# EavianWoo/SinGS

Hardware: AMD Instinct MI355X
Metric: rendered views/sec fwd+bwd, 200k Gaussians @1080p (higher is better)
Workload: dtype f32; 1 GPU; S(200000,1920,1080,deg=3,seed=3): 200000 Gaussians, 1920x1080, SH deg 3, fwd+bwd, R=780064 (tile,Gaussian) pairs, every view of a step within 0.1 % of that (cameras a few cm apart), frame-parallel dp1; gaussians=200000, width=1920, height=1080, sh_degree=3, num_rendered=780064, tile_list_max=135, frames_per_launch=8, streams=2, regularisers=False, forward_only=False, hip_graph=False, reduction=fold of 2 gradient row(s) for 16 views + collective in 1 chunk(s), gradient_rows=2, parallelism=dp1

## Files before the change

include/sings_hip.h:

```cpp
#ifndef SINGS_HIP_H
#define SINGS_HIP_H

#include <stddef.h>
#include <stdint.h>

#ifdef __cplusplus
extern "C" {
#endif

#define SG_TILE 16
#define SG_GRAD_REC_FLOATS 9

typedef struct SgRasterSettings {
    int32_t image_height;
    int32_t image_width;
    float tanfovx;
    float tanfovy;
    float scale_modifier;
    int32_t sh_degree;
    int32_t sh_coeffs;
    int32_t prefiltered;
    int32_t debug;
    int32_t flags;
    const float *bg;
// ... 347 lines not shown
int sg_init_attributes(int V, int F, int E, float init_scale_multiplier, float thickness_factor, const float *verts,
                       const int32_t *faces, const int32_t *edges, void *ws, int32_t *first, int32_t *second, float *scales,
                       float *scales_aux, float *normals, float *rotmat, int32_t *info, void *stream);
size_t sg_attr_mse_ws_bytes(void);
int sg_attr_mse(int N, const float *const *outputs, const float *const *targets, float *const *grads, void *ws, float *terms,
                void *stream);
int sg_plateau_step(int n_groups, int begin, int patience, const double *settings, const float *loss, double *state, float *hyper,
                    const float *terms, int n_copy, double *log, int log_rows, void *stream);

#define SG_NUM_KERNELS 8
enum SgKernelId {
    SG_K_PREPROCESS_FWD = 0, SG_K_PHOTO_LOSS = 1, SG_K_TILE_SCAN = 2, SG_K_TILE_SCATTER = 3,
    SG_K_TILE_SORT = 4, SG_K_RENDER_FWD = 5, SG_K_RENDER_BWD = 6, SG_K_PREPROCESS_BWD = 7
};
int sg_profile_enable(int on);
int sg_copy_probe(void *dst, const void *src, size_t bytes, int non_temporal, void *stream);
int sg_profile_collect(double *total_ms, int64_t *launches, int n);
const char *sg_kernel_name(int id);

#ifdef __cplusplus
}
#endif
#endif
```

sings_amd/_lib.py:

```python
import ctypes as C
import os

_HERE = os.path.dirname(os.path.abspath(__file__))
LIB_PATH = os.environ.get("SINGS_HIP_LIB") or os.path.join(_HERE, "libsings_hip.so")
_lib = None


class SgRasterSettings(C.Structure):
    _fields_ = [
        ("image_height", C.c_int32), ("image_width", C.c_int32),
        ("tanfovx", C.c_float), ("tanfovy", C.c_float), ("scale_modifier", C.c_float),
        ("sh_degree", C.c_int32), ("sh_coeffs", C.c_int32),
        ("prefiltered", C.c_int32), ("debug", C.c_int32), ("flags", C.c_int32),
        ("bg", C.c_void_p), ("viewmatrix", C.c_void_p), ("projmatrix", C.c_void_p), ("campos", C.c_void_p),
        ("count_signal", C.c_void_p), ("count_signal_host", C.c_void_p),
    ]


class SgLayout(C.Structure):
    _fields_ = [(n, C.c_size_t) for n in (
        "geom_recA", "geom_recB", "geom_recC", "geom_depth", "geom_flags", "geom_slot", "geom_bytes",
        "bin_header", "bin_tile_count", "bin_ranges", "bin_cursor", "bin_pair_keys", "bin_point_list",
        "bin_point_keys", "bin_pair_gid", "bin_pair_tile", "bin_pair_local", "bin_sort_items", "bin_rank_items", "bin_items", "bin_ck_start", "bin_plan", "bin_pair_mask", "bin_item_w", "bin_item_perm", "bin_rec_valid", "bin_tile_keys", "bin_bytes", "img_final_T", "img_n_contrib", "img_ckpt", "img_bytes", "bwd_bytes")]

# ... 115 lines not shown
    "sg_mesh_edges_build": "i: i2 p5",
    "sg_mesh_edges_emit": "i: i3 p7",
    "sg_mesh_subdivide": "i: i3 p6",
    "sg_mesh_midpoints": "i: i3 p4",
    "sg_mesh_midpoints_i32": "i: i3 p4",
    "sg_mesh_collapse_max_edges": "i:",
    "sg_mesh_collapse_ws_bytes": "z: i2",
    "sg_mesh_collapse_build": "i: i3 p3 d p3",
    "sg_mesh_collapse_emit": "i: i4 p6",
    "sg_init_ws_bytes": "z: i",
    "sg_init_attributes": "i: i3 f2 p12",
    "sg_attr_mse_ws_bytes": "z:",
    "sg_attr_mse": "i: i V3 p3",
    "sg_plateau_step": "i: i3 d p4 i p i p",
    "sg_profile_enable": "i: i",
    "sg_copy_probe": "i: p2 z i p",
    "sg_profile_collect": "i: d n i",
    "sg_kernel_name": "s: i",
}
_P = C.POINTER
_CTYPE = {"i": C.c_int, "z": C.c_size_t, "f": C.c_float, "s": C.c_char_p,
          "p": C.c_void_p,
          "S": _P(SgRasterSettings), "F": _P(SgFrameBatch), "K": _P(SgSkinInputs), "L": _P(SgLayout), "T": _P(SgTriplane),
          "D": _P(SgLinearSide),
          "n": _P(C.c_int64), "Z": _P(C.c_size_t), "d": _P(C.c_double),
          "V": _P(C.c_void_p),
          "G": _P(C.c_void_p * 3 * 4)}
EXPORTS = tuple(_PROTOTYPES)
LPIPS_NUM_OFFSETS = 46
LPIPS_WS_NUM_PIECES = 28
# ... 64 lines not shown
```

sings_amd/csrc/sg_api.hip:

```cpp
#include "sg_common.h"

#include <chrono>
#include <stdarg.h>
#include <stdio.h>
#include <stdlib.h>
#include <thread>
#include <string.h>
#include <utility>
#include <vector>

static thread_local char g_err[512] = "";

static int sg_fail(const char *what, hipError_t e)
{
    snprintf(g_err, sizeof g_err, "%s: %s", what, e == hipSuccess ? "invalid argument" : hipGetErrorString(e));
    return 1;
}

static int sg_failf(const char *fmt, ...)
{
    char msg[256];
    va_list ap;
    va_start(ap, fmt);
    vsnprintf(msg, sizeof msg, fmt, ap);
// ... 1153 lines not shown
    if (!g_prof_on) return;
    hipEvent_t e;
    (void)hipEventCreate(&e);
    (void)hipEventRecord(e, st);
    g_prof_open[id] = e;
}
void sg_prof_end(int id, hipStream_t st)
{
    if (!g_prof_on) return;
    hipEvent_t e;
    (void)hipEventCreate(&e);
    (void)hipEventRecord(e, st);
    g_prof_ev[id].push_back(std::make_pair(g_prof_open[id], e));
}
extern "C" int sg_profile_enable(int on) { g_prof_on = on != 0; return 0; }
extern "C" int sg_profile_collect(double *total_ms, int64_t *launches, int n)
{
    if (!total_ms || !launches || n < SG_NUM_KERNELS) return sg_fail("sg_profile_collect", hipSuccess);
    hipError_t e = hipDeviceSynchronize();
    if (e != hipSuccess) return sg_fail("sg_profile_collect", e);
    for (int k = 0; k < SG_NUM_KERNELS; k++) {
        for (auto &p : g_prof_ev[k]) {
            float ms = 0;
            (void)hipEventElapsedTime(&ms, p.first, p.second);
            total_ms[k] += ms; launches[k] += 1;
            (void)hipEventDestroy(p.first); (void)hipEventDestroy(p.second);
        }
        g_prof_ev[k].clear();
    }
    return 0;
// ... 9 lines not shown
```

sings_amd/csrc/sg_common.h:

```cpp
#pragma once
#include <hip/hip_runtime.h>
#include <stdint.h>
#include <stddef.h>

#include "../../include/sings_hip.h"

#define SG_WAVE 64
int sg_set_error(const char *what, hipError_t e = hipSuccess);
#ifdef SG_EXP
#error "SG_EXP experiment variants were removed from the product sources"
#endif
#define SG_MAX_TILES (1u << 20)
#define SG_SEG 256
__host__ __device__ inline uint32_t sg_nseg(uint32_t n) { return n > SG_SEG && n <= SG_SEG * 4095u ? (n + SG_SEG - 1) / SG_SEG : 0u; }
__host__ __device__ inline uint32_t sg_items_cap(size_t T, size_t cap) { size_t v = T + cap / SG_SEG + 2; return v > 0xffffffffull ? 0xffffffffu : (uint32_t)v; }
__host__ __device__ inline uint32_t sg_group_slots(uint32_t n) { return n > 1024u ? 6u * ((n + 1023u) / 1024u) + 2u : 0u; }
__host__ __device__ inline uint32_t sg_sort_items_cap(size_t T, size_t cap) { size_t v = (T < cap / 1024 ? T : cap / 1024) + 2; return v > 0xffffffffull ? 0xffffffffu : (uint32_t)v; }
__host__ __device__ inline uint32_t sg_rank_items_cap(size_t cap) { size_t v = cap / 73 + 16; return v > 0xffffffffull ? 0xffffffffu : (uint32_t)v; }
__host__ __device__ inline uint32_t sg_ckpt_cap(size_t cap) { size_t v = 2 * (cap / SG_SEG) + 2; return v > 0xffffffffull ? 0xffffffffu : (uint32_t)v; }
__host__ __device__ inline uint32_t sg_ctr_blocks_x(uint32_t gx) { return (gx + 3u) >> 2; }
__host__ __device__ inline size_t sg_ctr_count(uint32_t gx, uint32_t gy) { return (size_t)sg_ctr_blocks_x(gx) * ((gy + 3u) >> 2) * 16u; }
__host__ __device__ inline uint32_t sg_ctr_index(uint32_t tx, uint32_t ty, uint32_t gx)
{
    return ((ty >> 2) * sg_ctr_blocks_x(gx) + (tx >> 2)) * 16u + ((ty & 3u) << 2) + (tx & 3u);
// ... 184 lines not shown
struct SgCam {
    int W, H, gx, gy, flags;
    float tanfovx, tanfovy, fx, fy, mod;
    int D, M;
    const float *view, *proj, *campos, *bg;
    unsigned long long *count_signal;
};
__host__ __device__ __forceinline__ SgCam sg_frame(SgCam c, int frame, int cam_stride)
{
    const size_t f = (size_t)frame * (size_t)cam_stride;
    c.view += 16 * f; c.proj += 16 * f; c.campos += 3 * f;
    if (c.count_signal) c.count_signal += frame;
    return c;
}

void sg_launch_preprocess_fwd(const SgCam &c, const SgBatch &bt, int P, const float *means3D, const float *shs,
                              const float *colors_precomp, const float *opacities, const float *scales,
                              const float *rotations, const float *cov3D_precomp, SgGeom g, SgBin b,
                              size_t cap, int32_t *radii, hipStream_t st);
void sg_launch_binning(const SgCam &c, const SgBatch &bt, int P, const int32_t *radii, SgGeom g, SgBin b, size_t cap,
                       int write_keys, hipStream_t st);
static inline uint32_t sg_cap32(size_t cap) { return cap > 0xffffffffull ? 0xffffffffu : (uint32_t)cap; }
void sg_launch_render_fwd(const SgCam &c, const SgBatch &bt, SgGeom g, SgBin b, size_t cap, SgImg im, float *out_color,
                          int write_keys, hipStream_t st, const SgAuxFwd *ax = nullptr);
void sg_launch_render_bwd(const SgCam &c, const SgBatch &bt, SgGeom g, SgBin b, size_t cap, SgImg im,
                          const float *dL_dpix, SgRec grec, hipStream_t st, const SgAuxBwd *ax = nullptr);
void sg_launch_record_sums(const SgBatch &bt, int P, const int32_t *radii, SgGeom g, SgRec grec, size_t cap, const uint32_t *header,
                           const uint8_t *rec_valid, float4 *a9out, hipStream_t st, const float *dz = nullptr, size_t dz_stride = 0);
static inline size_t sg_a9_bytes(int P, int K) { return K > 1 ? sg_align((size_t)K * (size_t)P * 48 + 256) : 0; }
void sg_launch_preprocess_bwd(const SgCam &c, const SgBatch &bt, int P, const float *means3D, const float *shs,
// ... 77 lines not shown
```

sings_amd/csrc/sg_render.hip:

```cpp
#include "sg_sort.h"

#define SG_FB 256
#define SG_BB 64
#define SG_UNSET 0xffffffffu

__device__ __forceinline__ float sg_exp(float x) { return __builtin_amdgcn_exp2f(x * 1.44269504088896340736f); }
#define SG_KA (-0.5f * 1.44269504088896340736f)
#define SG_KB (-1.44269504088896340736f)
__device__ __forceinline__ float sg_power2(float Ap, float Bp, float Cp, float dx, float dy)
{
    return fmaf(Cp * dy, dy, fmaf(Ap, dx, Bp * dy) * dx);
}

#define SG_XCD_RUN 16
__device__ __forceinline__ int sg_tile_of_block(int block)
{
    const int xcd = block & 7, slot = block >> 3;
    const int within = (slot + 7 * (slot >> 5)) & (SG_XCD_RUN - 1);
    return ((slot / SG_XCD_RUN) * 8 + xcd) * SG_XCD_RUN + within;
}

__device__ __forceinline__ float sg_min_q_rect(float A, float B, float C, float mx, float my, float x0, float x1,
                                               float y0, float y1)
{
    if (mx >= x0 && mx <= x1 && my >= y0 && my <= y1) return 0.0f;
    const float rA = __builtin_amdgcn_rcpf(A), rC = __builtin_amdgcn_rcpf(C);
    float best = 3.0e38f;
// ... 296 lines not shown

static inline int sg_render_blocks(int T) { return ((T + 8 * SG_XCD_RUN - 1) / (8 * SG_XCD_RUN)) * (8 * SG_XCD_RUN); }

void sg_launch_render_fwd(const SgCam &c, const SgBatch &bt, SgGeom g, SgBin b, size_t cap, SgImg im, float *out_color,
                          int write_keys, hipStream_t st, const SgAuxFwd *ax)
{
    static_assert(SG_FB == SG_SEG, "forward batches are the checkpoint granularity");
    const int T = c.gx * c.gy;
    const int grid = sg_render_blocks(T);
    const int grid4 = sg_render_blocks((T + 3) / 4);
    const unsigned K = (unsigned)bt.K;
    const bool few = sg_lds_hist(c.gx, c.gy);
    uint64_t *pk = write_keys ? b.point_keys : (uint64_t *)nullptr;
    const uint32_t key_pitch = sg_key_pitch(c.gx, c.gy, c.flags);
    const bool direct = key_pitch != 0u;
#define SG_RF_ARGS(NB) c.W, c.H, c.gx, T, NB, b.ranges, direct ? b.tile_keys : b.pair_keys, b.point_list, pk, g.recA, g.recB, g.recC, c.bg, out_color,     \
                       im.final_T, im.n_contrib, b.ck_start, im.ckpt, sg_ckpt_cap(cap), b.header, b.pair_mask, b.tile_count,       \
                       (const uint4 *)b.sort_items, sg_mask_plane(cap), b.plan, b.item_w, sg_items_cap((size_t)T, cap), key_pitch
    sg_prof_begin(SG_K_RENDER_FWD, st);
    if (ax && (K > 1 || (few && (c.flags & SG_FLAG_THROUGHPUT)))) {
        if (few) hipLaunchKernelGGL(sg_render_fwd_frames_aux_kernel<true>, dim3(grid, K), dim3(256), 0, st, bt, SG_RF_ARGS(grid), *ax);
        else hipLaunchKernelGGL(sg_render_fwd_frames_aux_kernel<false>, dim3(grid4, K), dim3(256), 0, st, bt, SG_RF_ARGS(grid4), *ax);
    } else if (ax) {
        if (few) {
            const int extra = sg_split_long(c.gx, c.gy, c.flags) ? 3 * (int)sg_sort_items_cap(T, cap) : 0;
            hipLaunchKernelGGL(sg_render_fwd_deep_aux_kernel, dim3(extra + grid), dim3(256), 0, st, SG_RF_ARGS(extra), *ax);
        } else
            hipLaunchKernelGGL(sg_render_fwd_aux_kernel, dim3(grid), dim3(256), 0, st, SG_RF_ARGS(grid), *ax);
    } else if (K > 1 || (few && (c.flags & SG_FLAG_THROUGHPUT))) {
        if (few) hipLaunchKernelGGL(sg_render_fwd_frames_kernel<true>, dim3(grid, K), dim3(256), 0, st, bt, SG_RF_ARGS(grid));
        else hipLaunchKernelGGL(sg_render_fwd_frames_kernel<false>, dim3(grid4, K), dim3(256), 0, st, bt, SG_RF_ARGS(grid4));
    } else if (few) {
        const int extra = sg_split_long(c.gx, c.gy, c.flags) ? 3 * (int)sg_sort_items_cap(T, cap) : 0;
        hipLaunchKernelGGL(sg_render_fwd_deep_kernel, dim3(extra + grid), dim3(256), 0, st, SG_RF_ARGS(extra));
    } else
        hipLaunchKernelGGL(sg_render_fwd_kernel, dim3(grid), dim3(256), 0, st, SG_RF_ARGS(grid));
    sg_prof_end(SG_K_RENDER_FWD, st);
#undef SG_RF_ARGS
}

#define SG_DPP(v, ctrl) __builtin_bit_cast(float, __builtin_amdgcn_update_dpp(0, __builtin_bit_cast(int, v), ctrl, 0xF, 0xF, false))

__device__ __forceinline__ float sg_reduce9(float v[9], int lane, float *v8tot)
{
    float a0 = v[0], a1 = v[1], a2 = v[2], a3 = v[3], a4 = v[4], a5 = v[5], a6 = v[6], a7 = v[7];
    asm volatile("s_nop 1\n\tv_permlane32_swap_b32 %0, %1\n\tv_permlane32_swap_b32 %2, %3\n\t"
// ... 20 lines not shown
}
__device__ __forceinline__ float sg_reduce_to63(float x)
{
    x += SG_DPP(x, 0xB1); x += SG_DPP(x, 0x4E); x += SG_DPP(x, 0x141); x += SG_DPP(x, 0x140);
    asm volatile("s_nop 1\n\tv_add_f32_dpp %0, %0, %0 row_bcast:15 row_mask:0xa\n\ts_nop 1\n\t"
                 "v_add_f32_dpp %0, %0, %0 row_bcast:31 row_mask:0xc" : "+v"(x));
    return x;
}
__device__ __forceinline__ int sg_red_idx(int lane)
{
    const int row = lane >> 4, half = (lane >> 3) & 1;
    const int base = row == 0 ? 0 : (row == 1 ? 2 : (row == 2 ? 1 : 3));
    return base + 4 * half;
}

#define SG_BWD_EVAL(KPOS, SKIP)                                                                                       \
                                     \
    const float dx = ga.x - pxf, dy = ga.y - pyf;                                                                     \
    const float power = sg_power2(ga.z, ga.w, gb.x, dx, dy);            \
    const float G = __builtin_amdgcn_exp2f(power);                                                                    \
    const float alpha = fminf(0.99f, gb.y * G);                                                                       \
    const bool valid = ((KPOS) < ncq_b) & !(power > 0.0f) & !(alpha < 1.0f / 255.0f);                                 \
    if (__ballot(valid) == 0ull) SKIP;                   \
    const float ae = valid ? alpha : 0.0f;                                                                            \
    const float rinv = __builtin_amdgcn_rcpf(1.0f - ae);                                     \
    Tr = Tr * rinv;                                                                     \
    const float dchan = ae * Tr;                                                                                      \
                         \
    const float e = (AUX ? fmaf(gz, dD, fmaf(gc, d2, fmaf(gb.w, d1, gb.z * d0))) : fmaf(gc, d2, fmaf(gb.w, d1, gb.z * d0))) - Sd; \
    Sd = fmaf(ae, e, Sd);                                                                                             \
    const float dLa = fmaf(-tb, rinv, e * Tr);                        \
    const float w = valid ? G * dLa : 0.0f;                          \
         \
          \
    do { } while (0)
#define SG_BWD_PARTIALS(V)                                                                                            \
    const float wx = w * dx, wy = w * dy;                                                                             \
// ... 104 lines not shown
#include "sg_render_bwd.inc"
#undef SG_BWD_AUX
#define SG_BWD_AUX 1
#include "sg_render_bwd.inc"
#undef SG_BWD_AUX

void sg_launch_render_bwd(const SgCam &c, const SgBatch &bt, SgGeom g, SgBin b, size_t cap, SgImg im,
                          const float *dL_dpix, SgRec grec, hipStream_t st, const SgAuxBwd *ax)
{
    static_assert(SG_SEG % SG_BB == 0, "segments are whole backward batches");
    const int T = c.gx * c.gy;
    const int grid = sg_render_blocks((int)sg_items_cap((size_t)T, cap));
    const int grid4 = sg_render_blocks((int)((sg_items_cap((size_t)T, cap) + 3u) / 4u));
    const unsigned K = (unsigned)bt.K;
    uint32_t cap32 = cap > 0xffffffffull ? 0xffffffffu : (uint32_t)cap;
    sg_prof_begin(SG_K_RENDER_BWD, st);
    if (sg_lds_hist(c.gx, c.gy)) {
        hipLaunchKernelGGL(sg_order_items_kernel, dim3(1, K), dim3(256), 0, st, bt, b.header, b.item_w, b.item_perm);
        if (ax)
        hipLaunchKernelGGL(sg_render_bwd_sparse_aux_kernel, dim3(grid, K), dim3(256), 0, st, bt, c.W, c.H, c.gx, T, grid, b.ranges,
                           b.point_list, g.recA, g.recB, g.recC, c.bg, im.final_T, im.n_contrib, dL_dpix,
                           grec.a, grec.b, cap32, b.header, b.items, b.ck_start, im.ckpt, sg_ckpt_cap(cap), b.pair_mask, sg_mask_plane(cap),
                           sg_split_long(c.gx, c.gy, c.flags) ? 1 : 0, b.item_perm, b.rec_valid, *ax);
        else
        hipLaunchKernelGGL(sg_render_bwd_sparse_kernel, dim3(grid, K), dim3(256), 0, st, bt, c.W, c.H, c.gx, T, grid, b.ranges,
                           b.point_list, g.recA, g.recB, g.recC, c.bg, im.final_T, im.n_contrib, dL_dpix,
                           grec.a, grec.b, cap32, b.header, b.items, b.ck_start, im.ckpt, sg_ckpt_cap(cap), b.pair_mask, sg_mask_plane(cap),
                           sg_split_long(c.gx, c.gy, c.flags) ? 1 : 0, b.item_perm, b.rec_valid);
    } else if (ax)
    hipLaunchKernelGGL(sg_render_bwd_aux_kernel, dim3(grid4, K), dim3(256), 0, st, bt, c.W, c.H, c.gx, T, grid4, b.ranges,
                       b.point_list, g.recA, g.recB, g.recC, c.bg, im.final_T, im.n_contrib, dL_dpix,
                       grec.a, grec.b, cap32, b.header, b.items, b.ck_start, im.ckpt, sg_ckpt_cap(cap), b.pair_mask, sg_mask_plane(cap),
                       sg_split_long(c.gx, c.gy, c.flags) ? 1 : 0, *ax);
    else
    hipLaunchKernelGGL(sg_render_bwd_kernel, dim3(grid4, K), dim3(256), 0, st, bt, c.W, c.H, c.gx, T, grid4, b.ranges,
                       b.point_list, g.recA, g.recB, g.recC, c.bg, im.final_T, im.n_contrib, dL_dpix,
                       grec.a, grec.b, cap32, b.header, b.items, b.ck_start, im.ckpt, sg_ckpt_cap(cap), b.pair_mask, sg_mask_plane(cap),
                       sg_split_long(c.gx, c.gy, c.flags) ? 1 : 0);
    sg_prof_end(SG_K_RENDER_BWD, st);
}
```

sings_amd/csrc/sg_render_bwd.inc:

```

#define SG_BWD_FIRST(A0, A1, A2, A3, A4, A5, A6, A7, A8, Wv, DX, DY, DC, C0, C1, C2)                                   \
    "v_mul_f32 " A0 ", " Wv ", " DX "\n\tv_mul_f32 " A1 ", " Wv ", " DY "\n\t"                                          \
    "v_mul_f32 " A2 ", " A0 ", " DX "\n\tv_mul_f32 " A3 ", " A0 ", " DY "\n\tv_mul_f32 " A4 ", " A1 ", " DY "\n\t"       \
    "v_mov_b32 " A5 ", " Wv "\n\t"                                                                                    \
    "v_mul_f32 " A6 ", " DC ", " C0 "\n\tv_mul_f32 " A7 ", " DC ", " C1 "\n\tv_mul_f32 " A8 ", " DC ", " C2 "\n\t"
#define SG_BWD_LATER(A0, A1, A2, A3, A4, A5, A6, A7, A8, T0, T1, Wv, DX, DY, DC, C0, C1, C2)                           \
    "v_mul_f32 " T0 ", " Wv ", " DX "\n\tv_mul_f32 " T1 ", " Wv ", " DY "\n\t"                                          \
    "v_add_f32 " A0 ", " A0 ", " T0 "\n\tv_add_f32 " A1 ", " A1 ", " T1 "\n\t"                                          \
    "v_fmac_f32 " A2 ", " T0 ", " DX "\n\tv_fmac_f32 " A3 ", " T0 ", " DY "\n\tv_fmac_f32 " A4 ", " T1 ", " DY "\n\t"    \
    "v_add_f32 " A5 ", " A5 ", " Wv "\n\t"                                                                            \
    "v_fmac_f32 " A6 ", " DC ", " C0 "\n\tv_fmac_f32 " A7 ", " DC ", " C1 "\n\tv_fmac_f32 " A8 ", " DC ", " C2 "\n\t"
#define SG_BWD_ACC9 "+v"(acc[0]), "+v"(acc[1]), "+v"(acc[2]), "+v"(acc[3]), "+v"(acc[4]), "+v"(acc[5]), "+v"(acc[6]), "+v"(acc[7]), "+v"(acc[8])
#define SG_BWD_ASSIGN()                                                                                               \
    do {                                                                                                              \
        if (AUX)                                                                                                      \
            asm volatile(SG_BWD_FIRST("%0", "%1", "%2", "%3", "%4", "%5", "%6", "%7", "%8", "%10", "%11", "%12", "%13", "%14", "%15", "%16") \
                         "v_mul_f32 %9, %13, %17"                                                                     \
                         : SG_BWD_ACC9, "+v"(acc[9]) : "v"(w), "v"(dx), "v"(dy), "v"(dchan), "v"(d0), "v"(d1), "v"(d2), "v"(dD)); \
        else                                                                                                          \
            asm volatile(SG_BWD_FIRST("%0", "%1", "%2", "%3", "%4", "%5", "%6", "%7", "%8", "%9", "%10", "%11", "%12", "%13", "%14", "%15") \
                         : SG_BWD_ACC9 : "v"(w), "v"(dx), "v"(dy), "v"(dchan), "v"(d0), "v"(d1), "v"(d2));             \
    } while (0)
#define SG_BWD_ASSIGN_OR_ADD()                                                                                        \
    do {                                                                                                              \
// ... 3 lines not shown
                         SG_BWD_LATER("%0", "%1", "%2", "%3", "%4", "%5", "%6", "%7", "%8", "%10", "%11", "%12", "%13", "%14", "%15", "%16", "%17", "%18") \
                         "v_fmac_f32 %9, %15, %19\n\ts_branch 2f\n1:\n\t"                                            \
                         SG_BWD_FIRST("%0", "%1", "%2", "%3", "%4", "%5", "%6", "%7", "%8", "%12", "%13", "%14", "%15", "%16", "%17", "%18") \
                         "v_mul_f32 %9, %15, %19\n2:"                                                                  \
                         : SG_BWD_ACC9, "+v"(acc[9]), "=&v"(t0), "=&v"(t1)                                             \
                         : "v"(w), "v"(dx), "v"(dy), "v"(dchan), "v"(d0), "v"(d1), "v"(d2), "v"(dD), "s"(some) : "scc"); \
        else                                                                                                          \
            asm volatile("s_cmp_lg_u32 %18, 0\n\ts_cbranch_scc0 1f\n\t"                                              \
                         SG_BWD_LATER("%0", "%1", "%2", "%3", "%4", "%5", "%6", "%7", "%8", "%9", "%10", "%11", "%12", "%13", "%14", "%15", "%16", "%17") \
                         "s_branch 2f\n1:\n\t"                                                                        \
                         SG_BWD_FIRST("%0", "%1", "%2", "%3", "%4", "%5", "%6", "%7", "%8", "%11", "%12", "%13", "%14", "%15", "%16", "%17") \
                         "\n2:"                                                                                       \
                         : SG_BWD_ACC9, "=&v"(t0), "=&v"(t1)                                                          \
                         : "v"(w), "v"(dx), "v"(dy), "v"(dchan), "v"(d0), "v"(d1), "v"(d2), "s"(some) : "scc");        \
    } while (0)
#define SG_BWD_QUAD(Q)                                                                                                \
    do {                                                                                                              \
        const float pxf = ((Q) & 1) ? pxf0 + 8.0f : pxf0, pyf = ((Q) >> 1) ? pyf0 + 8.0f : pyf0;                      \
        const float d0 = d04[Q], d1 = d14[Q], d2 = d24[Q], dD = dD4[Q], tb = tb4[Q];                                  \
        const uint32_t ncq_b = ncq4[Q];                                                                               \
        float &Tr = Tr4[Q], &Sd = Sd4[Q];                                                                             \
        SG_BWD_EVAL((uint32_t)pos, break);                            \
        if ((Q) == 0) SG_BWD_ASSIGN(); else SG_BWD_ASSIGN_OR_ADD();                                                   \
        some = 1u;                                                                                                    \
    } while (0)
__global__ void __launch_bounds__(256) __attribute__((amdgpu_waves_per_eu(SG_BWD_TW_WAVES, SG_BWD_TW_WAVES)))
#if SG_BWD_AUX
sg_render_bwd_aux_kernel(SG_BWD_PARAMS, SgAuxBwd ax)
#else
sg_render_bwd_kernel(SG_BWD_PARAMS)
#endif
{
    constexpr bool AUX = SG_BWD_AUX;
#if !SG_BWD_AUX
    const SgAuxBwd ax = { };
#endif
    __shared__ float4 sR[4][SG_BB][4];
    __shared__ float sG[4][SG_BB][9 + AUX];
    SG_STAMP_SCOPE
    SG_BWD_FRAME_OFFSETS;
#if SG_BWD_AUX
    SG_BWD_AUX_FRAME_OFFSETS;
#endif
    (void)T; (void)nblocks;
    const int nitems = header[1] ? 0 : (int)header[5];
    const int tid = threadIdx.x, lane = tid & 63;
    const int wave = __builtin_amdgcn_readfirstlane(tid >> 6);
    const int it = 4 * sg_tile_of_block(blockIdx.x) + wave;
    if (it >= nitems) return;
    const uint32_t item = items[it];
    const int tile = (int)(item & 0xfffffu), seg = (int)(item >> 20);
    const int tx = tile % gx, ty = tile / gx;
    const int X0 = tx * 16, Y0 = ty * 16;
    const uint2 range = ranges[tile];
    const int n = (int)(range.y - range.x);
    const uint32_t cks = ck_start[tile];
    const int lo = seg * SG_SEG;
    const int hi = cks != 0xffffffffu && lo + SG_SEG < n ? lo + SG_SEG : n;
    if (lo >= n) return;
// ... 25 lines not shown
            }
        }
        Tr4[q] = Tr; Sd4[q] = Sd; d04[q] = d0; d14[q] = d1; d24[q] = d2; dD4[q] = dD; ncq4[q] = ncq;
        uint32_t m = ncq;
#pragma unroll
        for (int o = 32; o > 0; o >>= 1) { uint32_t u = __shfl_xor(m, o, 64); m = u > m ? u : m; }
        maxq4[q] = (int)__builtin_amdgcn_readfirstlane(m);
    }
    const int max_contrib = max(max(maxq4[0], maxq4[1]), max(maxq4[2], maxq4[3]));
    const float ddelx_dx = 0.5f * (float)W, ddely_dy = 0.5f * (float)H;
    const int cslot = lane == 63 ? 8 : sg_red_idx(lane);
    float acc[10] = { };
    for (int base = lo + (hi - 1 - lo) / SG_BB * SG_BB; base >= lo; base -= SG_BB) {
        const int cnt = hi - base < SG_BB ? hi - base : SG_BB;
        uint32_t mk = 0u;
        if (lane < cnt) {
            const int e = base + lane;
            const uint32_t gid = point_list[range.x + e];
            if (e < max_contrib) {
                mk = pair_mask[range.x + e];
                if (split_long && n > SG_WSORT_MAX)
                    mk = (mk & 1u) | (pair_mask[(size_t)mask_plane + range.x + e] & 2u) | (pair_mask[2 * (size_t)mask_plane + range.x + e] & 4u) |
                         (pair_mask[3 * (size_t)mask_plane + range.x + e] & 8u);
                mk &= 15u;
            }
            const float4 c4 = recC[SG_REC_STRIDE * (size_t)gid];
            if (mk) {
                const float4 a = recA[SG_REC_STRIDE * (size_t)gid], b = recB[SG_REC_STRIDE * (size_t)gid];
                sR[wave][lane][0] = make_float4(a.x, a.y, SG_KA * a.z, SG_KB * a.w);
                sR[wave][lane][1] = make_float4(SG_KA * b.x, b.y, b.z, b.w);
                sR[wave][lane][2] = make_float4(c4.x, AUX ? ax.depth[gid] : 0.0f, __uint_as_float(mk), 0.0f);
                sR[wave][lane][3] = make_float4(a.z, a.w, b.x, 0.0f);
            }
            const uint32_t goff = __float_as_uint(c4.y), mn = __float_as_uint(c4.z), wh = __float_as_uint(c4.w);
            const int x0 = mn & 0xffff, y0 = mn >> 16, rw = wh & 0xffff;
            sR[wave][lane][3].w = __uint_as_float(goff + (uint32_t)((ty - y0) * rw + (tx - x0)));
        }
        unsigned long long todo = __ballot(mk != 0u);
        unsigned long long filed = 0ull;
        __builtin_amdgcn_s_waitcnt(0xC07F);
        __builtin_amdgcn_wave_barrier();
        while (todo) {
            const int k = 63 - __builtin_clzll(todo);
            todo &= ~(1ull << k);
            const int pos = base + k;
            const float4 ga = sR[wave][k][0], gb = sR[wave][k][1], gm = sR[wave][k][2];
            const float gc = gm.x, gz = gm.y;
            uint32_t mke = __builtin_amdgcn_readfirstlane(__float_as_uint(gm.z));
            if (pos >= maxq4[0]) mke &= ~1u;
            if (pos >= maxq4[1]) mke &= ~2u;
            if (pos >= maxq4[2]) mke &= ~4u;
            if (pos >= maxq4[3]) mke &= ~8u;
            uint32_t some = 0u;
            if (mke & 1u) SG_BWD_QUAD(0);
            if (mke & 2u) SG_BWD_QUAD(1);
            if (mke & 4u) SG_BWD_QUAD(2);
            if (mke & 8u) SG_BWD_QUAD(3);
            __builtin_amdgcn_wave_barrier();
            if (some) {
                SG_BWD_FILE(acc, acc[9], k);
                filed |= 1ull << k;
            }
        }
        __builtin_amdgcn_s_waitcnt(0xC07F);
        __builtin_amdgcn_wave_barrier();
        const float4 cn = sR[wave][lane][3];
        const uint32_t rslot = lane < cnt ? __float_as_uint(cn.w) : 0xffffffffu;
        if (rslot < cap) {
            float4 r0 = make_float4(0.0f, 0.0f, 0.0f, 0.0f), r1 = r0;
            float r2 = 0.0f, r3 = 0.0f;
            if ((filed >> lane) & 1ull) {
                float s[9 + AUX];
#pragma unroll
                for (int q = 0; q < 9 + AUX; q++) s[q] = sG[wave][lane][q];
                const float no = -sR[wave][lane][1].y, nh = 0.5f * no;
                const float m0 = fmaf(cn.x, s[0], cn.y * s[1]), m1 = fmaf(cn.y, s[0], cn.z * s[1]);
                r0 = make_float4(no * ddelx_dx * m0, no * ddely_dy * m1, nh * s[2], nh * s[3]);
                r1 = make_float4(nh * s[4], s[5], s[6], s[7]);
                r2 = s[8];
                if (AUX) r3 = s[9];
            }
            grec_a[2 * (size_t)rslot] = r0;
            grec_a[2 * (size_t)rslot + 1] = r1;
            grec_b[rslot] = r2;
            if (AUX) ax.dz[rslot] = r3;
        }
        __builtin_amdgcn_wave_barrier();
    }
}

#undef SG_BWD_QUAD
#undef SG_BWD_ASSIGN_OR_ADD
#undef SG_BWD_ASSIGN
#undef SG_BWD_ACC9
#undef SG_BWD_LATER
#undef SG_BWD_FIRST

__global__ void __launch_bounds__(256) __attribute__((amdgpu_waves_per_eu(6, 6)))
#if SG_BWD_AUX
sg_render_bwd_sparse_aux_kernel(SG_BWD_PARAMS, const uint32_t *__restrict__ perm, uint8_t *__restrict__ rec_valid, SgAuxBwd ax)
#else
sg_render_bwd_sparse_kernel(SG_BWD_PARAMS, const uint32_t *__restrict__ perm, uint8_t *__restrict__ rec_valid)
#endif
{
    constexpr bool AUX = SG_BWD_AUX;
// ... 133 lines not shown
```

sings_amd/csrc/sg_render_fwd.inc:

```

#define SG_TW_BATCH 64
#define SG_TWSORT_MAX 512
static_assert(SG_TWSORT_MAX * 8 == SG_TW_BATCH * 64 && SG_RANKSORT_MAX * 2 * 8 <= SG_TW_BATCH * 64, "sort buffers alias the wave's rows");
static_assert(SG_FB % SG_TW_BATCH == 0, "boxes and checkpoints are refreshed between batches");

#define SG_FWD_TW_QUAD(Q)                                                                                  \
    do {                                                                                                   \
        const float dx = ga.x - (((Q) & 1) ? pxf1 : pxf0), dy = ga.y - (((Q) >> 1) ? pyf1 : pyf0);         \
        const float power = sg_power2(ga.z, ga.w, gb.x, dx, dy);                                           \
        const float alpha = fminf(0.99f, gb.y * __builtin_amdgcn_exp2f(power));                            \
        const float test_T = Tr4[Q] * (1.0f - alpha);                                                      \
        const unsigned long long valid = __ballot(!(power > 0.0f)) & __ballot(!(alpha < 1.0f / 255.0f)) & ~dn4[Q]; \
        const unsigned long long term = valid & __ballot(test_T < 0.0001f);                                \
        const bool blend = __builtin_amdgcn_inverse_ballot_w64(valid & ~term);                             \
        const float w = blend ? alpha * Tr4[Q] : 0.0f;                                                     \
        C04[Q] = fmaf(gb.z, w, C04[Q]); C14[Q] = fmaf(gb.w, w, C14[Q]); C24[Q] = fmaf(gm.x, w, C24[Q]);    \
        if (AUX) Dz4[Q] = fmaf(gm.y, w, Dz4[Q]);                                                           \
        Tr4[Q] = blend ? test_T : Tr4[Q];                                                                  \
        last4[Q] = blend ? pos1 : last4[Q];                                                                \
        dn4[Q] |= term;                                                                                    \
    } while (0)

__device__ __forceinline__ float sg_uniform(float x) { return __uint_as_float(__builtin_amdgcn_readfirstlane(__float_as_uint(x))); }

__device__ __forceinline__ uint32_t sg_list_id(const uint32_t *p) { return __hip_atomic_load(p, __ATOMIC_RELAXED, __HIP_MEMORY_SCOPE_AGENT); }

template <bool AUX>
__device__ __forceinline__ void sg_render_fwd_tile_wave(SG_FWD_PARAMS, SgAuxFwd ax = SgAuxFwd{})
{
    __shared__ float4 sR[4][SG_TW_BATCH][4];
    (void)nblocks; (void)long_items; (void)mask_plane; (void)plan; (void)item_w; (void)w_plane;
    const int tid = threadIdx.x, lane = tid & 63;
    const int wave = __builtin_amdgcn_readfirstlane(tid >> 6);
    if (tid == 0 && blockIdx.x == 0) header[2] = 0u;
    const int tile0 = 4 * sg_tile_of_block((int)blockIdx.x);
    if (tile0 >= T) return;
    const bool overflow = header[1] != 0u;
    {
        bool coop = false;
#pragma unroll
        for (int w = 0; w < 4; w++) {
            const uint2 r = ranges[tile0 + w < T ? tile0 + w : T - 1];
            const int nw = overflow ? 0 : (int)(r.y - r.x);
            coop |= nw > SG_TWSORT_MAX && nw <= SG_WSORT_MAX;
        }
        if (coop) {
// ... 66 lines not shown
            if ((dn4[0] & dn4[1] & dn4[2] & dn4[3]) == ~0ull) break;
            if (base > 0 && cks != 0xffffffffu && cks + (uint32_t)(base / SG_SEG) < ck_cap) {
                int ln = lane;
                asm volatile("" : "+v"(ln));
                const size_t slot = (size_t)(cks + (uint32_t)(base / SG_SEG)) * 256 + (uint32_t)ln;
#pragma unroll
                for (int q = 0; q < 4; q++)
                    if (dn4[q] != ~0ull) {
                        ckpt[slot + q * 64] = make_float4(Tr4[q], C04[q], C14[q], C24[q]);
                        if (AUX) ax.ckD[slot + q * 64] = Dz4[q];
                    }
            }
        }
        const int e = base + lane;
        uint32_t mk = 0u;
        if (e < n) {
            mk = sg_quad_mask(pa, pb, X0f, Y0f, box);
            row[lane][0] = make_float4(pa.x, pa.y, SG_KA * pa.z, SG_KB * pa.w);
            row[lane][1] = make_float4(SG_KA * pb.x, pb.y, pb.z, pb.w);
            row[lane][2] = make_float4(pc, pz, __uint_as_float(mk), 0.0f);
            pair_mask[range.x + e] = (uint8_t)mk;
        }
        if (e + SG_TW_BATCH < n) {
            const uint32_t gid = sg_list_id(point_list + range.x + e + SG_TW_BATCH);
            pa = recA[SG_REC_STRIDE * (size_t)gid]; pb = recB[SG_REC_STRIDE * (size_t)gid]; pc = recC[SG_REC_STRIDE * (size_t)gid].x;
            if (AUX) pz = ax.depth[gid];
        }
        unsigned long long todo = __ballot(mk != 0u);
        __builtin_amdgcn_wave_barrier();
        while (todo) {
            const int k = __builtin_ctzll(todo);
            todo &= todo - 1ull;
            const float4 ga = row[k][0], gb = row[k][1], gm = row[k][2];
            const uint32_t mke = __builtin_amdgcn_readfirstlane(__float_as_uint(gm.z));
            uint32_t pos1;
            asm volatile("v_mov_b32 %0, %1" : "=v"(pos1) : "s"(base + k + 1));
            if (mke & 1u) SG_FWD_TW_QUAD(0);
            if (mke & 2u) SG_FWD_TW_QUAD(1);
            if (mke & 4u) SG_FWD_TW_QUAD(2);
            if (mke & 8u) SG_FWD_TW_QUAD(3);
        }
        __builtin_amdgcn_wave_barrier();
    }
    const size_t hw = (size_t)H * W;
    const float bg0 = bg[0], bg1 = bg[1], bg2 = bg[2];
    int ln = lane;
    asm volatile("" : "+v"(ln));
#pragma unroll
    for (int q = 0; q < 4; q++) {
        if (cks < ck_cap) {
            ckpt[(size_t)cks * 256 + q * 64 + ln] = make_float4(Tr4[q], C04[q], C14[q], C24[q]);
            if (AUX) ax.ckD[(size_t)cks * 256 + q * 64 + ln] = Dz4[q];
        }
        const int px = X0 + (ln & 7) + 8 * (q & 1), py = Y0 + (ln >> 3) + 8 * (q >> 1);
        if (px < W && py < H) {
            const size_t pid = (size_t)py * W + px;
            final_T[pid] = Tr4[q];
            n_contrib[pid] = last4[q];
            out_color[pid] = fmaf(Tr4[q], bg0, C04[q]);
            out_color[hw + pid] = fmaf(Tr4[q], bg1, C14[q]);
            out_color[2 * hw + pid] = fmaf(Tr4[q], bg2, C24[q]);
            if (AUX) { ax.out_depth[pid] = Dz4[q]; ax.out_alpha[pid] = 1.0f - Tr4[q]; }
        }
    }
}

#undef SG_FWD_TW_QUAD
```

Before: 5319 views/s.

## Classify plain Gaussians to skip alpha clamp and power test in render loops

Each Gaussian entry is classified as 'plain' when its opacity, conic and mean values guarantee the alpha clamp to 0.99 and the positive-power test can never trigger. Plain entries run a specialised forward and backward inner loop without those checks, and the entry loop is reorganised into runs of plain entries split by general ones. A debug switch forces every entry down the general path. The saving is a few ALU ops and ballots per entry-quad, paid for with extra classification work, more complex loop control and larger code, with correctness resting on the classification bounds being tight.

```diff
diff --git a/include/sings_hip.h b/include/sings_hip.h
--- a/include/sings_hip.h
+++ b/include/sings_hip.h
@@ -385,6 +385,7 @@
     SG_K_TILE_SORT = 4, SG_K_RENDER_FWD = 5, SG_K_RENDER_BWD = 6, SG_K_PREPROCESS_BWD = 7
 };
 int sg_profile_enable(int on);
+int sg_debug_all_general(int on);
 int sg_copy_probe(void *dst, const void *src, size_t bytes, int non_temporal, void *stream);
 int sg_profile_collect(double *total_ms, int64_t *launches, int n);
 const char *sg_kernel_name(int id);
diff --git a/sings_amd/_lib.py b/sings_amd/_lib.py
--- a/sings_amd/_lib.py
+++ b/sings_amd/_lib.py
@@ -153,6 +153,7 @@
     "sg_attr_mse": "i: i V3 p3",
     "sg_plateau_step": "i: i3 d p4 i p i p",
     "sg_profile_enable": "i: i",
+    "sg_debug_all_general": "i: i",
     "sg_copy_probe": "i: p2 z i p",
     "sg_profile_collect": "i: d n i",
     "sg_kernel_name": "s: i",
diff --git a/sings_amd/csrc/sg_api.hip b/sings_amd/csrc/sg_api.hip
--- a/sings_amd/csrc/sg_api.hip
+++ b/sings_amd/csrc/sg_api.hip
@@ -1191,6 +1191,8 @@
     g_prof_ev[id].push_back(std::make_pair(g_prof_open[id], e));
 }
 extern "C" int sg_profile_enable(int on) { g_prof_on = on != 0; return 0; }
+bool g_sg_all_general = false;
+extern "C" int sg_debug_all_general(int on) { g_sg_all_general = on != 0; return 0; }
 extern "C" int sg_profile_collect(double *total_ms, int64_t *launches, int n)
 {
     if (!total_ms || !launches || n < SG_NUM_KERNELS) return sg_fail("sg_profile_collect", hipSuccess);
diff --git a/sings_amd/csrc/sg_common.h b/sings_amd/csrc/sg_common.h
--- a/sings_amd/csrc/sg_common.h
+++ b/sings_amd/csrc/sg_common.h
@@ -222,6 +222,7 @@
     return c;
 }
 
+extern bool g_sg_all_general;
 void sg_launch_preprocess_fwd(const SgCam &c, const SgBatch &bt, int P, const float *means3D, const float *shs,
                               const float *colors_precomp, const float *opacities, const float *scales,
                               const float *rotations, const float *cov3D_precomp, SgGeom g, SgBin b,
diff --git a/sings_amd/csrc/sg_render.hip b/sings_amd/csrc/sg_render.hip
--- a/sings_amd/csrc/sg_render.hip
+++ b/sings_amd/csrc/sg_render.hip
@@ -11,6 +11,24 @@
 {
     return fmaf(Cp * dy, dy, fmaf(Ap, dx, Bp * dy) * dx);
 }
+
+#define SG_PLAIN_OPACITY 0.98f
+#define SG_PLAIN_DET 1e-2f
+#define SG_PLAIN_CONIC_MIN 9.31322574615478515625e-10f
+#define SG_PLAIN_CONIC_MAX 1073741824.0f
+#define SG_PLAIN_MEAN_MIN 5.9604644775390625e-8f
+#define SG_PLAIN_MEAN_MAX 32768.0f
+__device__ __forceinline__ bool sg_entry_plain(float4 a, float4 b)
+{
+    const float A = a.z, B = a.w, C = b.x, o = b.y, ax = fabsf(a.x), ay = fabsf(a.y);
+    const float AC = A * C;
+    return (o >= 0.0f) & (o <= SG_PLAIN_OPACITY) & (A >= SG_PLAIN_CONIC_MIN) & (A <= SG_PLAIN_CONIC_MAX) &
+           (C >= SG_PLAIN_CONIC_MIN) & (C <= SG_PLAIN_CONIC_MAX) & (AC - B * B > SG_PLAIN_DET * AC) &
+           (ax <= SG_PLAIN_MEAN_MAX) & (ay <= SG_PLAIN_MEAN_MAX) & ((ax >= SG_PLAIN_MEAN_MIN) | (ax == 0.0f)) &
+           ((ay >= SG_PLAIN_MEAN_MIN) | (ay == 0.0f));
+}
+#define SG_MASK_PLAIN 16u
+#define SG_NBLOCKS_ALL_GENERAL 0x40000000
 
 #define SG_XCD_RUN 16
 __device__ __forceinline__ int sg_tile_of_block(int block)
@@ -337,13 +355,14 @@
     uint64_t *pk = write_keys ? b.point_keys : (uint64_t *)nullptr;
     const uint32_t key_pitch = sg_key_pitch(c.gx, c.gy, c.flags);
     const bool direct = key_pitch != 0u;
+    const int all_general = g_sg_all_general ? SG_NBLOCKS_ALL_GENERAL : 0;
 #define SG_RF_ARGS(NB) c.W, c.H, c.gx, T, NB, b.ranges, direct ? b.tile_keys : b.pair_keys, b.point_list, pk, g.recA, g.recB, g.recC, c.bg, out_color,     \
                        im.final_T, im.n_contrib, b.ck_start, im.ckpt, sg_ckpt_cap(cap), b.header, b.pair_mask, b.tile_count,       \
                        (const uint4 *)b.sort_items, sg_mask_plane(cap), b.plan, b.item_w, sg_items_cap((size_t)T, cap), key_pitch
     sg_prof_begin(SG_K_RENDER_FWD, st);
     if (ax && (K > 1 || (few && (c.flags & SG_FLAG_THROUGHPUT)))) {
         if (few) hipLaunchKernelGGL(sg_render_fwd_frames_aux_kernel<true>, dim3(grid, K), dim3(256), 0, st, bt, SG_RF_ARGS(grid), *ax);
-        else hipLaunchKernelGGL(sg_render_fwd_frames_aux_kernel<false>, dim3(grid4, K), dim3(256), 0, st, bt, SG_RF_ARGS(grid4), *ax);
+        else hipLaunchKernelGGL(sg_render_fwd_frames_aux_kernel<false>, dim3(grid4, K), dim3(256), 0, st, bt, SG_RF_ARGS(grid4 | all_general), *ax);
     } else if (ax) {
         if (few) {
             const int extra = sg_split_long(c.gx, c.gy, c.flags) ? 3 * (int)sg_sort_items_cap(T, cap) : 0;
@@ -352,7 +371,7 @@
             hipLaunchKernelGGL(sg_render_fwd_aux_kernel, dim3(grid), dim3(256), 0, st, SG_RF_ARGS(grid), *ax);
     } else if (K > 1 || (few && (c.flags & SG_FLAG_THROUGHPUT))) {
         if (few) hipLaunchKernelGGL(sg_render_fwd_frames_kernel<true>, dim3(grid, K), dim3(256), 0, st, bt, SG_RF_ARGS(grid));
-        else hipLaunchKernelGGL(sg_render_fwd_frames_kernel<false>, dim3(grid4, K), dim3(256), 0, st, bt, SG_RF_ARGS(grid4));
+        else hipLaunchKernelGGL(sg_render_fwd_frames_kernel<false>, dim3(grid4, K), dim3(256), 0, st, bt, SG_RF_ARGS(grid4 | all_general));
     } else if (few) {
         const int extra = sg_split_long(c.gx, c.gy, c.flags) ? 3 * (int)sg_sort_items_cap(T, cap) : 0;
         hipLaunchKernelGGL(sg_render_fwd_deep_kernel, dim3(extra + grid), dim3(256), 0, st, SG_RF_ARGS(extra));
@@ -403,13 +422,15 @@
     return base + 4 * half;
 }
 
-#define SG_BWD_EVAL(KPOS, SKIP)                                                                                       \
+#define SG_BWD_EVAL(KPOS, SKIP) SG_BWD_EVAL_CLASS(KPOS, SKIP, false)
+#define SG_BWD_EVAL_CLASS(KPOS, SKIP, PLAIN)                                                                          \
                                      \
     const float dx = ga.x - pxf, dy = ga.y - pyf;                                                                     \
     const float power = sg_power2(ga.z, ga.w, gb.x, dx, dy);            \
     const float G = __builtin_amdgcn_exp2f(power);                                                                    \
-    const float alpha = fminf(0.99f, gb.y * G);                                                                       \
-    const bool valid = ((KPOS) < ncq_b) & !(power > 0.0f) & !(alpha < 1.0f / 255.0f);                                 \
+    const float alpha = (PLAIN) ? gb.y * G : fminf(0.99f, gb.y * G);                                                  \
+    const bool valid = (PLAIN) ? ((KPOS) < ncq_b) & !(alpha < 1.0f / 255.0f)                                          \
+                               : ((KPOS) < ncq_b) & !(power > 0.0f) & !(alpha < 1.0f / 255.0f);                       \
     if (__ballot(valid) == 0ull) SKIP;                   \
     const float ae = valid ? alpha : 0.0f;                                                                            \
     const float rinv = __builtin_amdgcn_rcpf(1.0f - ae);                                     \
@@ -544,6 +565,7 @@
     const int grid4 = sg_render_blocks((int)((sg_items_cap((size_t)T, cap) + 3u) / 4u));
     const unsigned K = (unsigned)bt.K;
     uint32_t cap32 = cap > 0xffffffffull ? 0xffffffffu : (uint32_t)cap;
+    const int all_general = g_sg_all_general ? SG_NBLOCKS_ALL_GENERAL : 0;
     sg_prof_begin(SG_K_RENDER_BWD, st);
     if (sg_lds_hist(c.gx, c.gy)) {
         hipLaunchKernelGGL(sg_order_items_kernel, dim3(1, K), dim3(256), 0, st, bt, b.header, b.item_w, b.item_perm);
@@ -558,12 +580,12 @@
                            grec.a, grec.b, cap32, b.header, b.items, b.ck_start, im.ckpt, sg_ckpt_cap(cap), b.pair_mask, sg_mask_plane(cap),
                            sg_split_long(c.gx, c.gy, c.flags) ? 1 : 0, b.item_perm, b.rec_valid);
     } else if (ax)
-    hipLaunchKernelGGL(sg_render_bwd_aux_kernel, dim3(grid4, K), dim3(256), 0, st, bt, c.W, c.H, c.gx, T, grid4, b.ranges,
+    hipLaunchKernelGGL(sg_render_bwd_aux_kernel, dim3(grid4, K), dim3(256), 0, st, bt, c.W, c.H, c.gx, T, grid4 | all_general, b.ranges,
                        b.point_list, g.recA, g.recB, g.recC, c.bg, im.final_T, im.n_contrib, dL_dpix,
                        grec.a, grec.b, cap32, b.header, b.items, b.ck_start, im.ckpt, sg_ckpt_cap(cap), b.pair_mask, sg_mask_plane(cap),
                        sg_split_long(c.gx, c.gy, c.flags) ? 1 : 0, *ax);
     else
-    hipLaunchKernelGGL(sg_render_bwd_kernel, dim3(grid4, K), dim3(256), 0, st, bt, c.W, c.H, c.gx, T, grid4, b.ranges,
+    hipLaunchKernelGGL(sg_render_bwd_kernel, dim3(grid4, K), dim3(256), 0, st, bt, c.W, c.H, c.gx, T, grid4 | all_general, b.ranges,
                        b.point_list, g.recA, g.recB, g.recC, c.bg, im.final_T, im.n_contrib, dL_dpix,
                        grec.a, grec.b, cap32, b.header, b.items, b.ck_start, im.ckpt, sg_ckpt_cap(cap), b.pair_mask, sg_mask_plane(cap),
                        sg_split_long(c.gx, c.gy, c.flags) ? 1 : 0);
diff --git a/sings_amd/csrc/sg_render_bwd.inc b/sings_amd/csrc/sg_render_bwd.inc
--- a/sings_amd/csrc/sg_render_bwd.inc
+++ b/sings_amd/csrc/sg_render_bwd.inc
@@ -41,15 +41,38 @@
                          : SG_BWD_ACC9, "=&v"(t0), "=&v"(t1)                                                          \
                          : "v"(w), "v"(dx), "v"(dy), "v"(dchan), "v"(d0), "v"(d1), "v"(d2), "s"(some) : "scc");        \
     } while (0)
-#define SG_BWD_QUAD(Q)                                                                                                \
+#define SG_BWD_QUAD(Q, PLAIN)                                                                                         \
     do {                                                                                                              \
         const float pxf = ((Q) & 1) ? pxf0 + 8.0f : pxf0, pyf = ((Q) >> 1) ? pyf0 + 8.0f : pyf0;                      \
         const float d0 = d04[Q], d1 = d14[Q], d2 = d24[Q], dD = dD4[Q], tb = tb4[Q];                                  \
         const uint32_t ncq_b = ncq4[Q];                                                                               \
         float &Tr = Tr4[Q], &Sd = Sd4[Q];                                                                             \
-        SG_BWD_EVAL((uint32_t)pos, break);                            \
+        SG_BWD_EVAL_CLASS((uint32_t)pos, break, PLAIN);               \
         if ((Q) == 0) SG_BWD_ASSIGN(); else SG_BWD_ASSIGN_OR_ADD();                                                   \
         some = 1u;                                                                                                    \
+    } while (0)
+#define SG_BWD_ENTRY(PLAIN)                                                                                           \
+    do {                                                                                                              \
+        const int pos = base + k;                                        \
+        const float4 ga = sR[wave][k][0], gb = sR[wave][k][1], gm = sR[wave][k][2];                                   \
+        const float gc = gm.x, gz = gm.y;                                                                             \
+        uint32_t mke = __builtin_amdgcn_readfirstlane(__float_as_uint(gm.z));                                         \
+         \
+        if (pos >= maxq4[0]) mke &= ~1u;                                                                              \
+        if (pos >= maxq4[1]) mke &= ~2u;                                                                              \
+        if (pos >= maxq4[2]) mke &= ~4u;                                                                              \
+        if (pos >= maxq4[3]) mke &= ~8u;                                                                              \
+                                        \
+        uint32_t some = 0u;                  \
+        if (mke & 1u) SG_BWD_QUAD(0, PLAIN);                                                                          \
+        if (mke & 2u) SG_BWD_QUAD(1, PLAIN);                                                                          \
+        if (mke & 4u) SG_BWD_QUAD(2, PLAIN);                                                                          \
+        if (mke & 8u) SG_BWD_QUAD(3, PLAIN);                                                                          \
+        __builtin_amdgcn_wave_barrier();     \
+        if (some) {                                           \
+            SG_BWD_FILE(acc, acc[9], k);                                                                              \
+            filed |= 1ull << k;                                                                                       \
+        }                                                                                                             \
     } while (0)
 __global__ void __launch_bounds__(256) __attribute__((amdgpu_waves_per_eu(SG_BWD_TW_WAVES, SG_BWD_TW_WAVES)))
 #if SG_BWD_AUX
@@ -69,7 +92,8 @@
 #if SG_BWD_AUX
     SG_BWD_AUX_FRAME_OFFSETS;
 #endif
-    (void)T; (void)nblocks;
+    (void)T;
+    const bool all_general = (nblocks & SG_NBLOCKS_ALL_GENERAL) != 0;
     const int nitems = header[1] ? 0 : (int)header[5];
     const int tid = threadIdx.x, lane = tid & 63;
     const int wave = __builtin_amdgcn_readfirstlane(tid >> 6);
@@ -125,6 +149,7 @@
     for (int base = lo + (hi - 1 - lo) / SG_BB * SG_BB; base >= lo; base -= SG_BB) {
         const int cnt = hi - base < SG_BB ? hi - base : SG_BB;
         uint32_t mk = 0u;
+        bool plain = false;
         if (lane < cnt) {
             const int e = base + lane;
             const uint32_t gid = point_list[range.x + e];
@@ -140,7 +165,8 @@
                 const float4 a = recA[SG_REC_STRIDE * (size_t)gid], b = recB[SG_REC_STRIDE * (size_t)gid];
                 sR[wave][lane][0] = make_float4(a.x, a.y, SG_KA * a.z, SG_KB * a.w);
                 sR[wave][lane][1] = make_float4(SG_KA * b.x, b.y, b.z, b.w);
-                sR[wave][lane][2] = make_float4(c4.x, AUX ? ax.depth[gid] : 0.0f, __uint_as_float(mk), 0.0f);
+                plain = sg_entry_plain(a, b) & !all_general;
+                sR[wave][lane][2] = make_float4(c4.x, AUX ? ax.depth[gid] : 0.0f, __uint_as_float(plain ? mk | SG_MASK_PLAIN : mk), 0.0f);
                 sR[wave][lane][3] = make_float4(a.z, a.w, b.x, 0.0f);
             }
             const uint32_t goff = __float_as_uint(c4.y), mn = __float_as_uint(c4.z), wh = __float_as_uint(c4.w);
@@ -148,29 +174,24 @@
             sR[wave][lane][3].w = __uint_as_float(goff + (uint32_t)((ty - y0) * rw + (tx - x0)));
         }
         unsigned long long todo = __ballot(mk != 0u);
+        unsigned long long gen = __ballot(mk != 0u && !plain);
         unsigned long long filed = 0ull;
         __builtin_amdgcn_s_waitcnt(0xC07F);
         __builtin_amdgcn_wave_barrier();
         while (todo) {
-            const int k = 63 - __builtin_clzll(todo);
-            todo &= ~(1ull << k);
-            const int pos = base + k;
-            const float4 ga = sR[wave][k][0], gb = sR[wave][k][1], gm = sR[wave][k][2];
-            const float gc = gm.x, gz = gm.y;
-            uint32_t mke = __builtin_amdgcn_readfirstlane(__float_as_uint(gm.z));
-            if (pos >= maxq4[0]) mke &= ~1u;
-            if (pos >= maxq4[1]) mke &= ~2u;
-            if (pos >= maxq4[2]) mke &= ~4u;
-            if (pos >= maxq4[3]) mke &= ~8u;
-            uint32_t some = 0u;
-            if (mke & 1u) SG_BWD_QUAD(0);
-            if (mke & 2u) SG_BWD_QUAD(1);
-            if (mke & 4u) SG_BWD_QUAD(2);
-            if (mke & 8u) SG_BWD_QUAD(3);
-            __builtin_amdgcn_wave_barrier();
-            if (some) {
-                SG_BWD_FILE(acc, acc[9], k);
-                filed |= 1ull << k;
+            const unsigned long long upto = gen ? ~0ull >> __builtin_clzll(gen) : 0ull;
+            unsigned long long run = todo & ~upto;
+            todo &= upto;
+            while (run) {
+                const int k = 63 - __builtin_clzll(run);
+                run &= ~(1ull << k);
+                SG_BWD_ENTRY(true);
+            }
+            if (todo) {
+                const int k = 63 - __builtin_clzll(todo);
+                todo &= ~(1ull << k);
+                gen &= ~(1ull << k);
+                SG_BWD_ENTRY(false);
             }
         }
         __builtin_amdgcn_s_waitcnt(0xC07F);
@@ -200,6 +221,7 @@
     }
 }
 
+#undef SG_BWD_ENTRY
 #undef SG_BWD_QUAD
 #undef SG_BWD_ASSIGN_OR_ADD
 #undef SG_BWD_ASSIGN
diff --git a/sings_amd/csrc/sg_render_fwd.inc b/sings_amd/csrc/sg_render_fwd.inc
--- a/sings_amd/csrc/sg_render_fwd.inc
+++ b/sings_amd/csrc/sg_render_fwd.inc
@@ -4,13 +4,14 @@
 static_assert(SG_TWSORT_MAX * 8 == SG_TW_BATCH * 64 && SG_RANKSORT_MAX * 2 * 8 <= SG_TW_BATCH * 64, "sort buffers alias the wave's rows");
 static_assert(SG_FB % SG_TW_BATCH == 0, "boxes and checkpoints are refreshed between batches");
 
-#define SG_FWD_TW_QUAD(Q)                                                                                  \
+#define SG_FWD_TW_QUAD(Q, PLAIN)                                                                           \
     do {                                                                                                   \
         const float dx = ga.x - (((Q) & 1) ? pxf1 : pxf0), dy = ga.y - (((Q) >> 1) ? pyf1 : pyf0);         \
         const float power = sg_power2(ga.z, ga.w, gb.x, dx, dy);                                           \
-        const float alpha = fminf(0.99f, gb.y * __builtin_amdgcn_exp2f(power));                            \
+        const float alpha = (PLAIN) ? gb.y * __builtin_amdgcn_exp2f(power) : fminf(0.99f, gb.y * __builtin_amdgcn_exp2f(power)); \
         const float test_T = Tr4[Q] * (1.0f - alpha);                                                      \
-        const unsigned long long valid = __ballot(!(power > 0.0f)) & __ballot(!(alpha < 1.0f / 255.0f)) & ~dn4[Q]; \
+        const unsigned long long valid = (PLAIN) ? __ballot(!(alpha < 1.0f / 255.0f)) & ~dn4[Q]            \
+                                                 : __ballot(!(power > 0.0f)) & __ballot(!(alpha < 1.0f / 255.0f)) & ~dn4[Q]; \
         const unsigned long long term = valid & __ballot(test_T < 0.0001f);                                \
         const bool blend = __builtin_amdgcn_inverse_ballot_w64(valid & ~term);                             \
         const float w = blend ? alpha * Tr4[Q] : 0.0f;                                                     \
@@ -21,6 +22,18 @@
         dn4[Q] |= term;                                                                                    \
     } while (0)
 
+#define SG_FWD_TW_ENTRY(PLAIN)                                                                             \
+    do {                                                                                                   \
+        const float4 ga = row[k][0], gb = row[k][1], gm = row[k][2];                                       \
+        const uint32_t mke = __builtin_amdgcn_readfirstlane(__float_as_uint(gm.z));                        \
+        uint32_t pos1;                                                                                     \
+        asm volatile("v_mov_b32 %0, %1" : "=v"(pos1) : "s"(base + k + 1));                                 \
+        if (mke & 1u) SG_FWD_TW_QUAD(0, PLAIN);                                                            \
+        if (mke & 2u) SG_FWD_TW_QUAD(1, PLAIN);                                                            \
+        if (mke & 4u) SG_FWD_TW_QUAD(2, PLAIN);                                                            \
+        if (mke & 8u) SG_FWD_TW_QUAD(3, PLAIN);                                                            \
+    } while (0)
+
 __device__ __forceinline__ float sg_uniform(float x) { return __uint_as_float(__builtin_amdgcn_readfirstlane(__float_as_uint(x))); }
 
 __device__ __forceinline__ uint32_t sg_list_id(const uint32_t *p) { return __hip_atomic_load(p, __ATOMIC_RELAXED, __HIP_MEMORY_SCOPE_AGENT); }
@@ -29,7 +42,8 @@
 __device__ __forceinline__ void sg_render_fwd_tile_wave(SG_FWD_PARAMS, SgAuxFwd ax = SgAuxFwd{})
 {
     __shared__ float4 sR[4][SG_TW_BATCH][4];
-    (void)nblocks; (void)long_items; (void)mask_plane; (void)plan; (void)item_w; (void)w_plane;
+    const bool all_general = (nblocks & SG_NBLOCKS_ALL_GENERAL) != 0;
+    (void)long_items; (void)mask_plane; (void)plan; (void)item_w; (void)w_plane;
     const int tid = threadIdx.x, lane = tid & 63;
     const int wave = __builtin_amdgcn_readfirstlane(tid >> 6);
     if (tid == 0 && blockIdx.x == 0) header[2] = 0u;
@@ -126,11 +140,12 @@
         }
         const int e = base + lane;
         uint32_t mk = 0u;
+        const bool plain = sg_entry_plain(pa, pb) & !all_general;
         if (e < n) {
             mk = sg_quad_mask(pa, pb, X0f, Y0f, box);
             row[lane][0] = make_float4(pa.x, pa.y, SG_KA * pa.z, SG_KB * pa.w);
             row[lane][1] = make_float4(SG_KA * pb.x, pb.y, pb.z, pb.w);
-            row[lane][2] = make_float4(pc, pz, __uint_as_float(mk), 0.0f);
+            row[lane][2] = make_float4(pc, pz, __uint_as_float(plain ? mk | SG_MASK_PLAIN : mk), 0.0f);
             pair_mask[range.x + e] = (uint8_t)mk;
         }
         if (e + SG_TW_BATCH < n) {
@@ -139,18 +154,23 @@
             if (AUX) pz = ax.depth[gid];
         }
         unsigned long long todo = __ballot(mk != 0u);
+        unsigned long long gen = __ballot(mk != 0u && !plain);
         __builtin_amdgcn_wave_barrier();
         while (todo) {
-            const int k = __builtin_ctzll(todo);
-            todo &= todo - 1ull;
-            const float4 ga = row[k][0], gb = row[k][1], gm = row[k][2];
-            const uint32_t mke = __builtin_amdgcn_readfirstlane(__float_as_uint(gm.z));
-            uint32_t pos1;
-            asm volatile("v_mov_b32 %0, %1" : "=v"(pos1) : "s"(base + k + 1));
-            if (mke & 1u) SG_FWD_TW_QUAD(0);
-            if (mke & 2u) SG_FWD_TW_QUAD(1);
-            if (mke & 4u) SG_FWD_TW_QUAD(2);
-            if (mke & 8u) SG_FWD_TW_QUAD(3);
+            const unsigned long long front = gen ? (gen & (0ull - gen)) - 1ull : ~0ull;
+            unsigned long long run = todo & front;
+            todo &= ~front;
+            while (run) {
+                const int k = __builtin_ctzll(run);
+                run &= run - 1ull;
+                SG_FWD_TW_ENTRY(true);
+            }
+            if (todo) {
+                const int k = __builtin_ctzll(todo);
+                todo &= todo - 1ull;
+                gen &= gen - 1ull;
+                SG_FWD_TW_ENTRY(false);
+            }
         }
         __builtin_amdgcn_wave_barrier();
     }
@@ -177,4 +197,5 @@
     }
 }
 
+#undef SG_FWD_TW_ENTRY
 #undef SG_FWD_TW_QUAD
```

Result: no change. 5338 views/s, median of 6 (+0.4%).
